# utiasSTARS/pyslam

Hardware: AMD Instinct MI355X
Metric: ms/LM-iter (Jac build + J^T J + Schur solve), stereo BA @ 500k residuals (lower is better)
Workload: dtype f64

## Files before the change

include/pyslam_hip.h:

```cpp
#ifndef PYSLAM_HIP_H
#define PYSLAM_HIP_H

#include <stdint.h>

#ifdef __cplusplus
extern "C" {
#endif

typedef struct ps_problem ps_problem;

typedef struct ps_problem_desc {
    int32_t dof;
    int32_t num_poses;
    const double*  poses;
    const int32_t* pose_rid;
    int32_t num_points;
    const double*  points;
    const int32_t* point_vid;

    int64_t num_obs;
    const int32_t* obs_pose;
    const int32_t* obs_point;
    const double*  obs_uvd;
    const int32_t* obs_grp;
// ... 138 lines not shown
                          double* dx, double* covariance );

int ps_sparse_normal_solve(int32_t m, int32_t n, const int32_t* j_row_ptr, const int32_t* j_col, const double* j_val,
                           const int32_t* jt_row_ptr, const int32_t* jt_col, const double* jt_val,
                           const double* r, const double* rhs, double tol, int32_t max_iters,
                           double* dx, int32_t* iters_out, double* relres_out);

int ps_sparse_normal_direct(int32_t m, int32_t n, const int32_t* j_row_ptr, const int32_t* j_col, const double* j_val,
                            const int32_t* jt_row_ptr, const int32_t* jt_col, const double* jt_val,
                            const double* r, const double* rhs, int32_t refine_steps, double* dx, double* relres_out);

int ps_debug_band_inverse(const double* a, int32_t ncb, int32_t dof, int32_t bw, int32_t chunk_nodes, float* ainv_out,
                          double* elapsed_us);
int ps_debug_factor_stress(const double* a, int32_t ncb, int32_t dof, int32_t bw, int32_t mode, int32_t launches, int32_t lowprio,
                           int32_t aggressor, int32_t* n_diff, int32_t* n_pivot);

int ps_ransac_transforms(const double* pts_1, const double* pts_2, int32_t batch, int32_t n, double* T_out);
int ps_ransac_cost(const double* T, int32_t num_hyp, const double* pts_1, const double* obs_2, int32_t num_pts,
                   const double* cam5, double thresh, uint8_t* masks, int32_t* counts);
int ps_ransac_frame_to_frame(const double* pts_1, const double* pts_2, const double* obs_2, int32_t num_pts,
                             const int32_t* sample_idx, int32_t num_hyp, int32_t set_size, const double* cam5,
                             double thresh, double* T_all, int32_t* counts, int32_t* best_index,
                             int32_t* best_count, double* T_best, uint8_t* best_mask);

typedef struct ps_photo ps_photo;
typedef struct ps_photo_desc {
    int32_t num_pixels;
    const double* pt_ref;
    const double* im_ref;
    const double* im_jac;
// ... 40 lines not shown
```

pyslam_amd/_native.py:

```python
import ctypes as C
import os

import numpy as np

_HERE = os.path.dirname(os.path.abspath(__file__))
LIB_PATH = os.path.join(_HERE, 'lib', 'libpyslam_hip.so')
if os.environ.get('PYSLAM_AMD_MEASURE') == '1':
    LIB_PATH = os.path.join(_HERE, 'lib', 'libpyslam_hip_measure.so')

c_i32p = C.POINTER(C.c_int32)
c_f64p = C.POINTER(C.c_double)
c_u8p = C.POINTER(C.c_uint8)
PS_NUM_STAGES = 12
STAGE_NAMES = ['landmark_pass', 'pose_pass', 'schur_pairs', 'pose_factors', 'pcg',
               'backsub', 'update', 'cost', 'iteration_total', 'cg_kernel', 'allreduce', 'pack_unpack']


class ProblemDesc(C.Structure):
    _fields_ = [
        ('dof', C.c_int32), ('num_poses', C.c_int32), ('poses', c_f64p), ('pose_rid', c_i32p),
        ('num_points', C.c_int32), ('points', c_f64p), ('point_vid', c_i32p),
        ('num_obs', C.c_int64), ('obs_pose', c_i32p), ('obs_point', c_i32p), ('obs_uvd', c_f64p),
        ('obs_grp', c_i32p),
        ('num_cams', C.c_int32), ('cams', c_f64p), ('num_stiff3', C.c_int32), ('stiff3', c_f64p),
# ... 104 lines not shown
    'ps_dense_make_tables': (C.c_int, [H, C.c_int32, C.c_int32, c_i32p, c_f64p, C.c_double, C.c_double, C.c_double]),
    'ps_dense_track': (C.c_int, [H, C.c_int32, C.c_int32, C.c_int32, c_i32p, c_i32p, C.POINTER(SolveOptions), C.c_int32,
                                 C.c_double, c_f64p, c_f64p, c_i32p, c_f64p, C.c_int32]),
    'ps_dense_level_shape': (C.c_int, [H, C.c_int32, c_i32p, c_i32p]),
    'ps_dense_read_level': (C.c_int, [H, C.c_int32, C.c_int32, C.c_int32, c_f64p]),
    'ps_dense_num_pixels': (C.c_int, [H, C.c_int32, C.c_int32, c_i32p]),
    'ps_dense_read_tables': (C.c_int, [H, C.c_int32, C.c_int32, C.c_int32, c_f64p, c_f64p, c_f64p, c_f64p]),
    'ps_dense_device_bytes': (C.c_int, [H, C.POINTER(C.c_int64)]),
    'ps_dense_normal_solve': (C.c_int, [c_f64p, c_f64p, C.c_int32, C.c_int32, c_f64p, c_f64p]),
    'ps_sparse_normal_solve': (C.c_int, [C.c_int32, C.c_int32, c_i32p, c_i32p, c_f64p, c_i32p, c_i32p, c_f64p, c_f64p, c_f64p,
                                         C.c_double, C.c_int32, c_f64p, c_i32p, c_f64p]),
    'ps_sparse_normal_direct': (C.c_int, [C.c_int32, C.c_int32, c_i32p, c_i32p, c_f64p, c_i32p, c_i32p, c_f64p, c_f64p, c_f64p,
                                          C.c_int32, c_f64p, c_f64p]),
    'ps_debug_band_inverse': (C.c_int, [c_f64p, C.c_int32, C.c_int32, C.c_int32, C.c_int32, C.POINTER(C.c_float), c_f64p]),
    'ps_debug_factor_stress': (C.c_int, [c_f64p, C.c_int32, C.c_int32, C.c_int32, C.c_int32, C.c_int32, C.c_int32, C.c_int32, c_i32p, c_i32p]),
}

_lib = None


class NativeError(RuntimeError):
    pass


def _share_torch_hip_runtime():
    import sys
    if 'torch' in sys.modules:
        return
    try:
        import importlib.util
# ... 83 lines not shown
```

pyslam_amd/csrc/ps_abi_problem.h:

```cpp


const char* ps_last_error(void) { return g_err.c_str(); }

int ps_device_count(void) {
    int n = 0;
    if (hipGetDeviceCount(&n) != hipSuccess) return 0;
    return n;
}

int ps_warm_up(void) {
    static std::once_flag once;
    static int rc = 0;
    std::call_once(once, [] {
        void* p = nullptr;
        if (hipMalloc(&p, 256) != hipSuccess) { rc = fail("hipMalloc failed (no usable HIP device?)"); return; }
        hipLaunchKernelGGL(k_zero4, dim3(1), dim3(256), 0, 0, (size_t)8, (double*)p, (size_t)0, (double*)nullptr, (size_t)0,
                           (double*)nullptr, (size_t)0, (double*)nullptr);
        double hostw[4] = {0, 0, 0, 0};
        (void)hipMemsetAsync(p, 0, 256, 0);
        (void)hipMemcpyAsync((char*)p + 128, p, 64, hipMemcpyDeviceToDevice, 0);
        (void)hipMemcpyAsync(hostw, p, sizeof(hostw), hipMemcpyDeviceToHost, 0);
        if (hipDeviceSynchronize() != hipSuccess) rc = fail("the warm-up launch failed");
        hipFree(p);
        hipFuncAttributes a;
#define PS_TOUCH(...) (void)hipFuncGetAttributes(&a, reinterpret_cast<const void*>(&__VA_ARGS__))
        PS_TOUCH(k_landmark_pass<false>); PS_TOUCH(k_landmark_pass_packed<false, false>); PS_TOUCH(k_landmark_pass_packed<false, true>); PS_TOUCH(k_backsub_packed); PS_TOUCH(k_pose_pass<false>); PS_TOUCH(k_pose_finalize); PS_TOUCH(k_schur_pairs_db<0>);
        PS_TOUCH(k_schur_combine); PS_TOUCH(k_backsub); PS_TOUCH(k_cost_reproj<false>); PS_TOUCH(k_cost_packed<false>); PS_TOUCH(k_reduce3); PS_TOUCH(k_reduce_partials);
        PS_TOUCH(k_copy2); PS_TOUCH(k_zero4); PS_TOUCH(k_lag_status_check);
        PS_TOUCH(k_block_jacobi_factor<6>); PS_TOUCH(k_scale_blocks<6>); PS_TOUCH(k_scale_blocks_p<6>); PS_TOUCH(k_rows_setup<6>);
        PS_TOUCH(k_coarse_rowsums<6>); PS_TOUCH(k_coarse_matrix<6>); PS_TOUCH(k_coarse_chol<6, true>); PS_TOUCH(k_coarse_border<6>);
        PS_TOUCH(k_coarse_mreduce<6>); PS_TOUCH(k_coarse_xbuild<6>); PS_TOUCH(k_coarse_recover<6>); PS_TOUCH(k_cg_fused_lds<6, 8>);
        PS_TOUCH(k_cg_fused<6, 8>); PS_TOUCH(k_cg_unscale<6>); PS_TOUCH(k_update_poses<6>); PS_TOUCH(k_update_points);
        PS_TOUCH(k_xcoarse_rowsums<6>); PS_TOUCH(k_xcoarse_matrix<6>); PS_TOUCH(k_band_chol<6>); PS_TOUCH(k_band_inverse); PS_TOUCH(k_band_inverse_rl<false>);
        PS_TOUCH(k_band_inverse_rl<true>); PS_TOUCH(k_bp_v); PS_TOUCH(k_bp_t); PS_TOUCH(k_bp_w); PS_TOUCH(k_bp_dense_sep); PS_TOUCH(k_bp_dense);
        PS_TOUCH(k_xcg_restrict<6>); PS_TOUCH(k_xcg_f2_coarse<6, 3>); PS_TOUCH(k_xcg_fused1<6, 8, false>); PS_TOUCH(k_xcg_fused1<6, 0, true>);
        PS_TOUCH(k_xcg_fused1<6, 2, false>); PS_TOUCH(k_xcg_fused1<6, 6, false>);
        PS_TOUCH(k_factor_pass<6>); PS_TOUCH(k_factor_assemble<6>); PS_TOUCH(k_cost_factors<6>);
        PS_TOUCH(k_factor_pass<3>); PS_TOUCH(k_factor_assemble<3>); PS_TOUCH(k_cost_factors<3>); PS_TOUCH(k_block_jacobi_factor<3>);
        PS_TOUCH(k_update_poses<3>); PS_TOUCH(k_direct_solve<6>); PS_TOUCH(k_direct_solve<3>);
        PS_TOUCH(k_motion_only_solve<false>); PS_TOUCH(k_motion_only_iteration<false>);
        PS_TOUCH(k_pcg_spmv<6>); PS_TOUCH(k_pcg_spmv<3>); PS_TOUCH(k_ldi_init); PS_TOUCH(k_ldi_update); PS_TOUCH(k_ldi_gemm); PS_TOUCH(k_ldi_mirror);
        PS_TOUCH(k_ldi_ritz); PS_TOUCH(k_ldi_seed_prep); PS_TOUCH(k_ldi_fro_total); PS_TOUCH(k_ldi_pad_identity);
        PS_TOUCH(k_ldi_scaled_dense<6>); PS_TOUCH(k_ldi_sym_unscale<6>); PS_TOUCH(k_ldi_scaled_dense<3>); PS_TOUCH(k_ldi_sym_unscale<3>);
        PS_TOUCH(k_shard_pack<6>); PS_TOUCH(k_shard_unpack<6>); PS_TOUCH(k_publish); PS_TOUCH(k_cov_rhs);
        PS_TOUCH(k_scale_blocks<3>); PS_TOUCH(k_rows_setup<3>); PS_TOUCH(k_coarse_rowsums<3>); PS_TOUCH(k_coarse_matrix<3>);
        PS_TOUCH(k_coarse_chol<3, true>); PS_TOUCH(k_coarse_border<3>); PS_TOUCH(k_coarse_mreduce<3>); PS_TOUCH(k_coarse_xbuild<3>);
        PS_TOUCH(k_coarse_recover<3>); PS_TOUCH(k_cg_fused_lds<3, 8>); PS_TOUCH(k_cg_unscale<3>);
#undef PS_TOUCH
    });
    return rc;
}

int ps_problem_destroy(ps_problem* h) {
    if (!h) return 0;
    if (h->cp_dbg) {
        long long c[8]; hipMemcpy(c, h->cp_dbg, 64, hipMemcpyDeviceToHost);
        int khz = 100000; hipDeviceGetAttribute(&khz, hipDeviceAttributeWallClockRate, 0);
        fprintf(stderr, "k_cg_persist, workgroup 0, %ld launches, us per launch: recurrences %.2f | sync %.2f | products + publish %.2f | gather %.2f "
                "(%.1f failed passes) | sync %.2f | dots + sync %.2f\n", h->cp_launches, c[0] * 1e3 / khz / h->cp_launches, c[1] * 1e3 / khz / h->cp_launches,
                c[2] * 1e3 / khz / h->cp_launches, c[3] * 1e3 / khz / h->cp_launches, (double)c[7] / h->cp_launches, c[4] * 1e3 / khz / h->cp_launches,
                c[5] * 1e3 / khz / h->cp_launches);
// ... 1058 lines not shown
```

pyslam_amd/csrc/ps_abi_small.h:

```cpp

int ps_ransac_transforms(const double* pts_1, const double* pts_2, int32_t batch, int32_t n, double* T_out) {
    if (!pts_1 || !pts_2 || !T_out || batch < 0 || n <= 0) return fail("bad argument");
    if (batch == 0) return 0;
    if (need_device()) return -1;
    const size_t nb = (size_t)batch * n * 3 * sizeof(double);
    DevBuf a, b, t;
    if (a.get(nb) || b.get(nb) || t.get((size_t)batch * 16 * sizeof(double))) return -1;
    HIP_OK(hipMemcpy(a.p, pts_1, nb, hipMemcpyHostToDevice));
    HIP_OK(hipMemcpy(b.p, pts_2, nb, hipMemcpyHostToDevice));
    hipLaunchKernelGGL(k_ransac_transforms, dim3(cdiv(batch, 64)), dim3(64), 0, 0, batch, n, a.as<double>(), b.as<double>(),
                       t.as<double>());
    HIP_OK(hipMemcpy(T_out, t.p, (size_t)batch * 16 * sizeof(double), hipMemcpyDeviceToHost));
    return 0;
}

int ps_ransac_cost(const double* T, int32_t num_hyp, const double* pts_1, const double* obs_2, int32_t num_pts,
                   const double* cam5, double thresh, uint8_t* masks, int32_t* counts) {
    if (!T || !pts_1 || !obs_2 || !cam5 || num_hyp < 0 || num_pts < 0) return fail("bad argument");
    if (num_hyp == 0) return 0;
    if (need_device()) return -1;
    DevBuf dT, dp, dobs, dcam, dcnt, dmask;
    const size_t pb = (size_t)num_pts * 3 * sizeof(double);
    if (dT.get((size_t)num_hyp * 16 * sizeof(double)) || dp.get(pb) || dobs.get(pb) || dcam.get(5 * sizeof(double)) ||
        dcnt.get((size_t)num_hyp * sizeof(int32_t)) || dmask.get((size_t)num_hyp * num_pts)) return -1;
// ... 438 lines not shown
                                    : bp->run<3>(st, bA.as<double>(), nc, bInv.as<float>(), nc, bst.as<int32_t>());
            HIP_OK(hipEventRecord(e1, st));
            if (rc) { bp.reset(); return -1; }
            if (rep == 1) { HIP_OK(hipStreamSynchronize(st)); bp.reset(); }
        }
        HIP_OK(hipStreamSynchronize(st));
    }
    HIP_OK(hipEventElapsedTime(&ms, e0, e1));
    if (elapsed_us) *elapsed_us = 1e3 * ms;
    int32_t stw[ST_NWORDS];
    HIP_OK(hipMemcpy(stw, bst.p, sizeof(stw), hipMemcpyDeviceToHost));
    HIP_OK(hipMemcpy(ainv_out, bInv.p, (size_t)nc * nc * 4, hipMemcpyDeviceToHost));
    if (stw[ST_DIAG_FAIL]) return fail("band factorisation: the matrix is not positive definite");
    return 0;
}
```

pyslam_amd/csrc/ps_abi_solver.h:

```cpp

int ps_get_info(ps_problem* h, ps_problem_info* info) {
    if (!h || !info) return fail("null argument");
    info->dof = h->D; info->num_poses = h->P; info->num_reduced = h->nr; info->num_points = h->L;
    info->num_var_points = h->nv; info->num_obs = h->N; info->num_edges = h->F; info->num_priors = 0;
    info->reduced_nnzb = h->nnzb; info->num_pairs = h->npairs;
    info->reduce_count = ((long)h->nnzb + h->nr) / 2 * h->D * h->D + (long)h->nr * h->D + 3;
    info->device_bytes = (int64_t)h->dev_bytes;
    info->cg_restarts = h->cg_fallbacks;
    info->cg_kernel_launches = h->cg_kernel_launches;
    info->ldi_solves = h->ldi_solves; info->ldi_fallbacks = h->ldi_fallbacks; info->ldi_seeds = h->ldi_seeds;
    info->xcg_fused_solves = h->xf_solves; info->xcg_fused_fallbacks = h->xf_fallbacks;
    info->cg_persist_solves = h->cp_launches; info->cg_persist_failures = h->cp_failures;
    info->cg_persist_refused = h->cp_refused; info->persist_cus = h->persist_cus;
    info->persist_cus_needed = h->cp_ok ? h->cp_cus_needed : (h->xp_ok ? h->xp_cus_needed : 0);
    info->landmark_passes_taken_over = h->prelm_used;
    info->xcg_persist4_solves = h->xp4_launches;
    return 0;
}

int ps_eval_cost(ps_problem* h, int include_all_constant, double* cost) {
    if (!h || !cost) return fail("null argument");
    if (include_all_constant && h->fuse_cost == 1 && lm_cost_possible(h)) { if (lm_cost_pass(h, h->lin_lambda, SC_COST)) return -1; }
    else if (cost_pass(h, include_all_constant, SC_COST)) return -1;
    if (read_scalars(h)) return -1;
// ... 747 lines not shown
    else if (n == "cg_ablate" || n == "schur_ablate" || n == "lm_ablate") {
        if (value != 0.0) return fail(n + ": timing experiments exist in the measurement build only (__graft_entry__.build_measure(), PYSLAM_AMD_MEASURE=1)");
    }
#endif
    else if (n == "schur_pipeline") h->schur_pipeline = value != 0.0;
    else if (n == "schur_mode") {
        if (value != 0.0 && value != 1.0) return fail("schur_mode must be 0 (gather kernels) or 1 (pose-stationary kernel)");
        if (value == 0.0 && !h->gather_lists) return fail("schur_mode 0: the gather kernels' pair lists were not built for this handle (create it under PS_SCHUR_MODE=0 or 2)");
        h->schur_mode = (int)value;
    }
    else if (n == "schur_stream") { if (value != 0.0 && !h->st_tiles) return fail("schur_stream: the streaming lists were not built for this problem"); h->use_stream = value != 0.0; }
    else if (n == "coarse_lag") h->coarse_lag = value != 0.0;
    else if (n == "cg_force_restart") h->cg_force_restart = value != 0.0;
    else if (n == "xcg_restrict_fused") h->xcg_rt = value != 0;
    else if (n == "band_chol") { h->band_chol = value != 0; h->lci_next = -1; }
    else if (n == "lm_packed") h->lm_packed = value != 0;
    else if (n == "pose_async") h->pose_async = (int)value;
    else if (n == "pose_xcd") h->pose_xcd = value != 0;
    else if (n == "xcg_persist4") h->xcg_persist4 = value != 0;
    else if (n == "cg_pipelined") { if (value != 0 && value != 1 && value != 2) return fail("cg_pipelined must be 0, 1 or 2"); h->cg_pipelined = (int)value; }
    else if (n == "fuse_cost") h->fuse_cost = (int)value;
    else if (n == "sync_refactor") h->sync_refactor = value != 0;
    else if (n == "hold_across_steps") h->hold_across_steps = value != 0;
    else if (n == "band_part") { h->band_part = value != 0; h->lci_next = -1; }
    else if (n == "band_part_chunk") { if (value < 0 || value > 4096) return fail("band_part_chunk must be 0 (automatic) .. 4096 nodes"); h->band_part_m = (int)value; h->lci_next = -1; }
    else if (n == "coarse_auto_hold") h->xcg_auto_hold = value != 0;
    else if (n == "coarse_adaptive_hold") h->xcg_adaptive_hold = value != 0;
    else if (n == "xcg_fused") { if (value != 0 && value != 1 && value != 2) return fail("xcg_fused must be 0, 1 or 2"); h->xcg_fused = (int)value; }
    else if (n == "lagged_inverse") { h->ldi_enable = value != 0; if (!h->ldi_enable) { h->ldi_cur = -1; if (h->ldi_state != 1) h->ldi_state = 0; } relook_path(h); }
    else if (n == "ldi_max_unknowns") { if (value < 0 || value > PS_LDI_MAXN) return fail("ldi_max_unknowns out of range (0 .. 3328)"); h->ldi_max_n = (int)value; relook_path(h); }
// ... 114 lines not shown
```

pyslam_amd/csrc/ps_core.hip:

```cpp
#include <hip/hip_runtime.h>

#include <algorithm>
#include <array>
#include <map>
#include <atomic>
#include <chrono>
#include <thread>
#include <climits>
#include <cmath>
#include <cstdio>
#include <cstring>
#include <memory>
#include <mutex>
#include <string>
#include <vector>

#include "pyslam_hip.h"
#include "ps_kernels.h"
#include "ps_ransac.h"
#include "ps_photo.h"
#include "ps_k_dense.h"
#include "ps_sparse.h"

namespace {
// ... 208 lines not shown
    bool side_pending = false;
    int coarse_lag = 1;
    hipStream_t side = nullptr;
    int side_cus = 0;
    hipEvent_t ev_ac = nullptr, ev_chol = nullptr, ev_acdone = nullptr;
    unsigned long long* chk_sums = nullptr; int chk_nsum = 0;
    double *chk_Ac = nullptr, *chk_BSZ = nullptr, *chk_Ac_side = nullptr; int32_t* chk_cnt = nullptr; size_t chk_bsz_n = 0;
    bool acdone_pending = false;
    int32_t* lag_status = nullptr;
    double* Mc = nullptr;
    bool mc_active = false;
    bool coarse_built = false;
    bool coarse_clamped = false;
    int cg_ablate = 0, schur_ablate = 0, lm_ablate = 0;
    int schur_pipeline = 1;
    int max_pose_obs = 0;
    int mo_fused = 1;
    double* mo_partials = nullptr;
    bool status_clean = true;
    int direct_fused = ps_env("PS_DIRECT_3LAUNCH") ? 0 : 1;
    int direct_max = 90;
    double *dA = nullptr, *dLi = nullptr, *dLiT = nullptr;
    int big_chol = 1;
    int explicit_ok = 1;
    bool cg_explicit = false;
    int xcg_refresh_every = 1;
    long xcg_lag_count = 0;
    int xcg_auto_hold = 1, xcg_held = 0;
    int xcg_adaptive_hold = 1;
    int xcg_its_ref = 0, xcg_good_held = 0;
// ... 300 lines not shown
```

pyslam_amd/csrc/ps_host_cg.h:

```cpp

namespace {

struct StageTimer {
    ps_problem* h;
    int stage;
    hipEvent_t a = nullptr, b = nullptr;
    int slot = -1;
    StageTimer(ps_problem* h_, int st, int level = 2) : h(h_), stage(st) {
        if (h->profiling < level) return;
        if (h->profiling == 1 && h->prof_every > 1 &&
            h->prof_tick % h->prof_every != (st == PS_ST_CG_KERNEL ? h->prof_every / 2 : 0)) return;
        if (h->ev_used + 2 > h->ev_pool.size()) {
            for (int i = 0; i < 64; ++i) { hipEvent_t e; hipEventCreate(&e); h->ev_pool.push_back(e); }
        }
        slot = (int)h->ev_used;
        a = h->ev_pool[h->ev_used++];
        b = h->ev_pool[h->ev_used++];
        hipEventRecord(a, h->stream);
    }
    void stop() {
        if (!a) return;
        hipEventRecord(b, h->stream);
        h->pending.push_back({stage, slot});
        a = nullptr;
// ... 480 lines not shown
    if (h->side_pending) { HIP_OK(hipStreamWaitEvent(h->stream, h->ev_chol, 0)); h->side_pending = false; }
    h->acdone_pending = false;
    h->lci_next = -1; h->lci_cur = 0; h->xcg_tag[0] = h->xcg_tag[1] = -1.0;
    if (ensure_cg_buffers(h, h->nr_aug, h->nnzb_aug)) return -1;
    HIP_OK(hipMemsetAsync(h->Saug, 0, (size_t)h->nnzb_aug * D * D * sizeof(double), h->stream));
    return 0;
}

inline void copy_doubles(hipStream_t st, double* dst, const double* src, size_t n) {
    if (!n) return;
    hipLaunchKernelGGL(k_copy2, dim3((unsigned)std::min<size_t>(2048, cdiv((long)n, 256))), dim3(256), 0, st, n, src, dst, (size_t)0,
                       (const double*)nullptr, (double*)nullptr);
}

template <int D>
int coarse_factor(ps_problem* h, hipStream_t st, int buf, int32_t* stat) {
    const int nc = h->nc, ncb = h->ncb;
    if (nc <= 90) {
        const size_t chol_lds = 2 * (size_t)nc * nc * sizeof(double);
        if (ensure_dynamic_lds((const void*)k_coarse_chol<D, true>, (size_t)(chol_lds))) return -1;
        hipLaunchKernelGGL((k_coarse_chol<D, true>), dim3(1), dim3(1024), chol_lds, st, ncb, h->Ac, h->Lci2[buf],
                           h->LciT2[buf], stat, nullptr);
    } else if (h->big_chol) {
        double* A = h->chol_scratch;
        double* Tinv = A + (size_t)nc * nc;
        copy_doubles(st, A, h->Ac, (size_t)nc * nc);
        const int nsteps = cdiv(nc, PS_BC_W);
        for (int s2 = 0; s2 < nsteps; ++s2) {
            const int j0 = s2 * PS_BC_W, w = std::min(PS_BC_W, nc - j0), m = nc - j0 - w;
            hipLaunchKernelGGL(k_bchol_panel, dim3(std::max(1, cdiv((long)m * w, 1024))), dim3(256), 0, st, nc, j0, A,
                               Tinv + (size_t)s2 * PS_BC_W * PS_BC_W, stat);
            if (m > 0) {
                const int nt = cdiv(m, 32);
                hipLaunchKernelGGL(k_bchol_update, dim3(nt * (nt + 1) / 2), dim3(256), 0, st, nc, j0, w, A);
            }
        }
        const bool dense_out = nc > PS_BI_S0 && !h->cg_explicit;
// ... 646 lines not shown
```

pyslam_amd/csrc/ps_host_iteration.h:

```cpp

namespace {

inline bool xcg_ac_on_main() { static const bool v = ps_env("PS_XCG_AC_MAIN") != nullptr; return v; }

template <int D>
void xcg_assemble_ac(ps_problem* h, hipStream_t st) {
    const int nr = h->nr, ncb = h->ncb;
    hipLaunchKernelGGL(k_xcoarse_rowsums<D>, dim3(nr), dim3(256), (size_t)(h->max_row_ents + 1) * D * D * sizeof(double), st,
                       nr, h->ent_ptr, h->ent_q, h->ent_lo, h->ent_hi, h->acol_idx, h->pnode, h->pw0, h->pw1, h->SB, h->Bmat, h->BSZ);
    hipLaunchKernelGGL(k_xcoarse_matrix<D>, dim3(cdiv((long)ncb * ncb * D * D, 256)), dim3(256), 0, st,
                       ncb, h->seg_ptr, h->seg_ent, h->seg_row, h->pnode, h->pw0, h->pw1, h->BSZ, h->Ac);
}

template <int D>
void xcg_launch(ps_problem* h, double tol, int count);

template <int D>
int xcg_setup(ps_problem* h, int max_iters, bool allow_lag) {
    const int nr = h->nr, ncb = h->ncb, nc = h->nc;
    if (max_iters + 2 > h->hist_cap) return fail("pcg max_iters exceeds the history buffer (4096)");
    if (h->acdone_pending) { HIP_OK(hipStreamWaitEvent(h->stream, h->ev_acdone, 0)); h->acdone_pending = false; }
    hipLaunchKernelGGL(k_block_jacobi_factor<D>, dim3(cdiv(nr, 4)), dim3(256), 0, h->stream, nr, h->diag_slot,
                       h->S, h->Linv, h->status, h->g, h->cg_r[0], h->cg_w[0], h->cg_s[0], h->cg_p, h->cg_xh,
                       h->poses, h->pose_of_rid, h->coarse_basis, h->Bmat, h->bgv);
// ... 336 lines not shown
int direct_solve_enqueue(ps_problem* h) {
    const int nr = h->nr, n = nr * D;
    if (h->direct_fused) {
        const size_t lds = ((size_t)n * n + 2 * (size_t)n + (size_t)nr * D * D) * sizeof(double);
        if (ensure_dynamic_lds((const void*)k_direct_solve<D>, lds)) return -1;
        static const int nt_env = ps_env("PS_DIRECT_THREADS") ? atoi(ps_env("PS_DIRECT_THREADS")) : 0;
        const int nthreads = nt_env > 0 ? nt_env : 1024;
        hipLaunchKernelGGL(k_direct_solve<D>, dim3(1), dim3(nthreads), lds, h->stream, nr, h->nnzb, h->brow_of, h->col_idx, h->S, h->g, h->x,
                           h->status, h->scalars);
        h->cg_launched = 0;
        return 0;
    }
    if (!h->dA && (h->alloc(&h->dA, (size_t)n * n) || h->alloc(&h->dLi, (size_t)n * n) || h->alloc(&h->dLiT, (size_t)n * n)))
        return -1;
    hipLaunchKernelGGL(k_bsr_to_dense<D>, dim3(1), dim3(256), 0, h->stream, nr, h->nnzb, h->brow_of, h->col_idx, h->S, h->dA);
    const size_t chol_lds = 2 * (size_t)n * n * sizeof(double);
    if (ensure_dynamic_lds((const void*)k_coarse_chol<D, true>, (size_t)(chol_lds))) return -1;
    hipLaunchKernelGGL((k_coarse_chol<D, true>), dim3(1), dim3(1024), chol_lds, h->stream, nr, h->dA, h->dLi, h->dLiT,
                       h->status, nullptr);
    hipLaunchKernelGGL(k_direct_apply<D>, dim3(1), dim3(256), 0, h->stream, n, h->dLi, h->dLiT, h->g, h->x, h->status,
                       h->scalars);
    h->cg_launched = 0;
    return 0;
}

int solve_reduced(ps_problem* h, double tol, int max_iters, int* iters, double* relres) {
    if (h->nr == 0) { if (iters) *iters = 0; if (relres) *relres = 0.0; return 0; }
    StageTimer t(h, PS_ST_PCG);
    if (use_direct(h)) {
        if (h->D == 6 ? direct_solve_enqueue<6>(h) : direct_solve_enqueue<3>(h)) return -1;
        if (read_scalars(h)) return -1;
        return cg_report(h, iters, relres);
    }
    if (h->pcg_variant == 1) {
// ... 161 lines not shown
```

pyslam_amd/csrc/ps_k_coarse.h:

```cpp
#pragma once


PS_DEV double coarse_weight(int j, int q, const int32_t* __restrict__ pnode,
                            const double* __restrict__ pw0, const double* __restrict__ pw1) {
    return (pnode[j] == q) ? pw0[j] : pw1[j];
}

template <int D>
__global__ __launch_bounds__(256) void k_coarse_rowsums(
    int nr, int ncb, const int32_t* __restrict__ run_lo, const int32_t* __restrict__ run_hi,
    const int32_t* __restrict__ acol_idx, const int32_t* __restrict__ pnode,
    const double* __restrict__ pw0, const double* __restrict__ pw1,
    const double* __restrict__ SB ,
    double* __restrict__ SZ, const double* __restrict__ Bmat, double* __restrict__ BSZ )
{
    constexpr int DD = D * D;
    extern __shared__ double srow[];
    const int i = blockIdx.x, nslot = ncb * DD;
    double* sBi = srow + nslot;
    if (threadIdx.x < DD) sBi[threadIdx.x] = Bmat[(size_t)i * DD + threadIdx.x];
    for (int t = threadIdx.x; t < nslot; t += blockDim.x) {
        const int q = t / DD, e = t % DD;
        const int k0 = run_lo[i * ncb + q], k1 = run_hi[i * ncb + q];
        double acc = 0.0;
// ... 68 lines not shown
    const int32_t* __restrict__ seg_row, const int32_t* __restrict__ pnode, const double* __restrict__ pw0,
    const double* __restrict__ pw1, const double* __restrict__ BSZ, double* __restrict__ Ac)
{
    constexpr int DD = D * D;
    const int nc = ncb * D;
    const int t = blockIdx.x * blockDim.x + threadIdx.x;
    if (t >= ncb * ncb * DD) return;
    const int e = t % DD, q2 = (t / DD) % ncb, q = t / (DD * ncb);
    double acc = 0.0;
    for (int s = seg_ptr[q * ncb + q2]; s < seg_ptr[q * ncb + q2 + 1]; ++s)
        acc += coarse_weight(seg_row[s], q, pnode, pw0, pw1) * BSZ[(size_t)seg_ent[s] * DD + e];
    Ac[(size_t)(q * D + e / D) * nc + q2 * D + e % D] = acc;
}

template <int D, bool IN_LDS>
__global__ __launch_bounds__(1024) void k_coarse_chol(int ncb, const double* __restrict__ A,
                                                       double* __restrict__ Li, double* __restrict__ LiT,
                                                       int32_t* __restrict__ status, double* gscratch)
{
    constexpr int DD = D * D;
    extern __shared__ __attribute__((aligned(16))) double sm[];
    const int nc = ncb * D;
    double* sL = IN_LDS ? sm : gscratch;
    double* sX = sL + nc * nc;
    __shared__ double sRl[64 * 6];
    const int t = threadIdx.x, nt = blockDim.x;
    for (int k = t; k < nc * nc; k += nt) { sL[k] = A[k]; sX[k] = 0.0; }
    auto factor_diag = [&](int J) {
        double a[D][D], rl[D];
        bool ok = true;
#pragma unroll
        for (int r = 0; r < D; ++r)
#pragma unroll
            for (int c = 0; c <= r; ++c) a[r][c] = sL[(J * D + r) * nc + J * D + c];
#pragma unroll
        for (int jj = 0; jj < D; ++jj) {
            double d = a[jj][jj];
#pragma unroll
            for (int k = 0; k < jj; ++k) d -= a[jj][k] * a[jj][k];
            if (!(d > 0.0)) { ok = false; d = 1.0; }
            rl[jj] = ps_rsqrt(d);
            a[jj][jj] = d * rl[jj];
#pragma unroll
            for (int r = jj + 1; r < D; ++r) {
                double v = a[r][jj];
#pragma unroll
                for (int k = 0; k < jj; ++k) v -= a[r][k] * a[jj][k];
                a[r][jj] = v * rl[jj];
            }
        }
        if (!ok) atomicAdd(&status[ST_DIAG_FAIL], 1);
#pragma unroll
        for (int r = 0; r < D; ++r) {
            sRl[J * D + r] = rl[r];
#pragma unroll
            for (int c = 0; c < D; ++c) sL[(J * D + r) * nc + J * D + c] = c <= r ? a[r][c] : 0.0;
        }
    };
    __syncthreads();
    if (t == 0) factor_diag(0);
    for (int J = 0; J < ncb; ++J) {
        __syncthreads();
        const int m = ncb - J - 1;
        for (int row = t; row < m * D; row += nt) {
            double* ar = sL + ((J + 1) * D + row) * nc + J * D;
            double x[D];
#pragma unroll
            for (int c = 0; c < D; ++c) {
                double v = ar[c];
#pragma unroll
                for (int k = 0; k < c; ++k) v -= x[k] * sL[(J * D + c) * nc + J * D + k];
                x[c] = v * sRl[J * D + c];
            }
#pragma unroll
            for (int c = 0; c < D; ++c) ar[c] = x[c];
        }
        __syncthreads();
        if (m == 0) break;
        if (t < 64) {
            if (t < DD) {
                const int a = t / D, b2 = t % D;
                double v = 0.0;
#pragma unroll
                for (int k = 0; k < D; ++k) v += sL[((J + 1) * D + a) * nc + J * D + k] * sL[((J + 1) * D + b2) * nc + J * D + k];
                sL[((J + 1) * D + a) * nc + (J + 1) * D + b2] -= v;
            }
            __builtin_amdgcn_wave_barrier();
            if (t == 0) factor_diag(J + 1);
        } else {
            for (int idx = t - 64; idx < m * m * DD; idx += nt - 64) {
                const int blk = idx / DD, e = idx % DD, a = e / D, b2 = e % D;
                const int I = J + 1 + blk / m, K = J + 1 + blk % m;
                if (K > I || (I == J + 1 && K == J + 1)) continue;
                double v = 0.0;
#pragma unroll
                for (int k = 0; k < D; ++k) v += sL[(I * D + a) * nc + J * D + k] * sL[(K * D + b2) * nc + J * D + k];
                sL[(I * D + a) * nc + K * D + b2] -= v;
            }
        }
    }
    __syncthreads();
    for (int k = t; k < ncb * D; k += nt) {
        const int R = k / D, c = k % D;
        double col[D];
#pragma unroll
        for (int r = 0; r < D; ++r) {
            double v = (r == c) ? 1.0 : 0.0;
#pragma unroll
            for (int q = 0; q < r; ++q) v -= (q >= c) ? sL[(R * D + r) * nc + R * D + q] * col[q] : 0.0;
            col[r] = (r >= c) ? v * sRl[R * D + r] : 0.0;
            sX[(R * D + r) * nc + R * D + c] = col[r];
        }
    }
    constexpr int NEX = IN_LDS ? 9 : 1;
    short ei[NEX], ej[NEX];
// ... 23 lines not shown
    };
    for (int sg = 1, lg = 1; sg < ncb; sg *= 2, ++lg) {
        __syncthreads();
        if (IN_LDS) {
#pragma unroll
            for (int u = 0; u < NEX; ++u) if (ei[u] >= 0) t_entry(ei[u], ej[u], sg, lg);
        } else for (int idx = t; idx < nc * nc; idx += nt) t_entry(idx / nc, idx % nc, sg, lg);
        __syncthreads();
        if (IN_LDS) {
#pragma unroll
            for (int u = 0; u < NEX; ++u) if (ei[u] >= 0) x_entry(ei[u], ej[u], sg, lg);
        } else for (int idx = t; idx < nc * nc; idx += nt) x_entry(idx / nc, idx % nc, sg, lg);
    }
    __syncthreads();
    for (int k = t; k < nc * nc; k += nt) {
        const int r = k / nc, c = k % nc;
        const double v = (c <= r) ? sX[k] : 0.0;
        Li[k] = v;
        LiT[(size_t)c * nc + r] = v;
    }
}

#define PS_BC_W 24
__global__ __launch_bounds__(256) void k_bchol_panel(
    int nc, int j0, double* __restrict__ A ,
    double* __restrict__ Tinv ,
    int32_t* __restrict__ status)
{
    __shared__ double sD[PS_BC_W * PS_BC_W], sI[PS_BC_W * PS_BC_W];
    const int t = threadIdx.x, w = min(PS_BC_W, nc - j0);
// ... 595 lines not shown
```

pyslam_amd/device.py:

```python
import ctypes as C

import numpy as np

from pyslam_amd import _native as nat


class DeviceProblem:
    def __init__(self, lp, stream=None, extra_pairs=None):
        lib = nat.require_gpu()
        self._lib = lib
        self.lp = lp
        self.dof = lp.dof
        d = nat.ProblemDesc()
        keep = []
        params_res = nat.is_resident(lp.poses)
        tables_res = nat.is_resident(lp.pose_rid)
        if params_res != nat.is_resident(lp.points):
            raise TypeError('poses and points must both be host arrays or both device tensors')
        d.flags = (nat.PS_DESC_DEVICE_PARAMS if params_res else 0) | (nat.PS_DESC_DEVICE_TABLES if tables_res else 0)

        def conv(a, np_dtype, want_res, to_ptr):
            if nat.is_resident(a) != want_res:
                raise TypeError('mixed host / device tables (ps_problem_desc.flags is per class: parameters, everything else)')
            if not want_res:
# ... 283 lines not shown
    cov = np.zeros((n, n)) if want_covariance else None
    nat.check(lib.ps_dense_normal_solve(nat.f64p(J), nat.f64p(r), m, n, nat.f64p(dx), nat.f64p(cov)))
    return (dx, cov) if want_covariance else dx


def band_inverse(A, ncb, dof, bw, chunk_nodes=0):
    lib = nat.require_gpu()
    A = np.ascontiguousarray(A, dtype=np.float64)
    n = ncb * dof
    assert A.shape == (n, n)
    out = np.zeros((n, n), dtype=np.float32)
    us = C.c_double(0.0)
    nat.check(lib.ps_debug_band_inverse(nat.f64p(A), ncb, dof, bw, chunk_nodes, out.ctypes.data_as(C.POINTER(C.c_float)),
                                        C.cast(C.byref(us), nat.c_f64p)))
    return out, us.value


class NotConverged(nat.NativeError):
    """The CG of the host-evaluated path stopped at max_iters with a residual too large to use."""


def sparse_normal_solve(J, r=None, rhs=None, tol=1e-12, max_iters=10000, accept=1e-6):
    lib = nat.require_gpu()
    J = J.tocsr()
    J.sort_indices()
    Jt = J.T.tocsr()
    Jt.sort_indices()
    m, n = J.shape
    a = [np.ascontiguousarray(x, dtype=t) for x, t in ((J.indptr, np.int32), (J.indices, np.int32), (J.data, np.float64),
                                                        (Jt.indptr, np.int32), (Jt.indices, np.int32), (Jt.data, np.float64))]
# ... 250 lines not shown
```

Baseline: 0.3034.

## Add fused coarse Cholesky kernel with precomputed thread mapping and fast inverse

```diff
diff --git a/include/pyslam_hip.h b/include/pyslam_hip.h
--- a/include/pyslam_hip.h
+++ b/include/pyslam_hip.h
@@ -176,6 +176,8 @@
                           double* elapsed_us);
 int ps_debug_factor_stress(const double* a, int32_t ncb, int32_t dof, int32_t bw, int32_t mode, int32_t launches, int32_t lowprio,
                            int32_t aggressor, int32_t* n_diff, int32_t* n_pivot);
+int ps_debug_coarse_chol(const double* a, int32_t ncb, int32_t dof, int32_t fused, int32_t repeats, double* li_out,
+                         int32_t* diag_fail, double* elapsed_us);
 
 int ps_ransac_transforms(const double* pts_1, const double* pts_2, int32_t batch, int32_t n, double* T_out);
 int ps_ransac_cost(const double* T, int32_t num_hyp, const double* pts_1, const double* obs_2, int32_t num_pts,
diff --git a/pyslam_amd/_native.py b/pyslam_amd/_native.py
--- a/pyslam_amd/_native.py
+++ b/pyslam_amd/_native.py
@@ -142,6 +142,7 @@
                                           C.c_int32, c_f64p, c_f64p]),
     'ps_debug_band_inverse': (C.c_int, [c_f64p, C.c_int32, C.c_int32, C.c_int32, C.c_int32, C.POINTER(C.c_float), c_f64p]),
     'ps_debug_factor_stress': (C.c_int, [c_f64p, C.c_int32, C.c_int32, C.c_int32, C.c_int32, C.c_int32, C.c_int32, C.c_int32, c_i32p, c_i32p]),
+    'ps_debug_coarse_chol': (C.c_int, [c_f64p, C.c_int32, C.c_int32, C.c_int32, C.c_int32, c_f64p, c_i32p, c_f64p]),
 }
 
 _lib = None
diff --git a/pyslam_amd/csrc/ps_abi_problem.h b/pyslam_amd/csrc/ps_abi_problem.h
--- a/pyslam_amd/csrc/ps_abi_problem.h
+++ b/pyslam_amd/csrc/ps_abi_problem.h
@@ -28,7 +28,7 @@
         PS_TOUCH(k_schur_combine); PS_TOUCH(k_backsub); PS_TOUCH(k_cost_reproj<false>); PS_TOUCH(k_cost_packed<false>); PS_TOUCH(k_reduce3); PS_TOUCH(k_reduce_partials);
         PS_TOUCH(k_copy2); PS_TOUCH(k_zero4); PS_TOUCH(k_lag_status_check);
         PS_TOUCH(k_block_jacobi_factor<6>); PS_TOUCH(k_scale_blocks<6>); PS_TOUCH(k_scale_blocks_p<6>); PS_TOUCH(k_rows_setup<6>);
-        PS_TOUCH(k_coarse_rowsums<6>); PS_TOUCH(k_coarse_matrix<6>); PS_TOUCH(k_coarse_chol<6, true>); PS_TOUCH(k_coarse_border<6>);
+        PS_TOUCH(k_coarse_rowsums<6>); PS_TOUCH(k_coarse_matrix<6>); PS_TOUCH(k_coarse_chol<6, true>); PS_TOUCH(k_coarse_chol_fs<6, false>); PS_TOUCH(k_coarse_border<6>);
         PS_TOUCH(k_coarse_mreduce<6>); PS_TOUCH(k_coarse_xbuild<6>); PS_TOUCH(k_coarse_recover<6>); PS_TOUCH(k_cg_fused_lds<6, 8>);
         PS_TOUCH(k_cg_fused<6, 8>); PS_TOUCH(k_cg_unscale<6>); PS_TOUCH(k_update_poses<6>); PS_TOUCH(k_update_points);
         PS_TOUCH(k_xcoarse_rowsums<6>); PS_TOUCH(k_xcoarse_matrix<6>); PS_TOUCH(k_band_chol<6>); PS_TOUCH(k_band_inverse); PS_TOUCH(k_band_inverse_rl<false>);
@@ -44,7 +44,7 @@
         PS_TOUCH(k_ldi_scaled_dense<6>); PS_TOUCH(k_ldi_sym_unscale<6>); PS_TOUCH(k_ldi_scaled_dense<3>); PS_TOUCH(k_ldi_sym_unscale<3>);
         PS_TOUCH(k_shard_pack<6>); PS_TOUCH(k_shard_unpack<6>); PS_TOUCH(k_publish); PS_TOUCH(k_cov_rhs);
         PS_TOUCH(k_scale_blocks<3>); PS_TOUCH(k_rows_setup<3>); PS_TOUCH(k_coarse_rowsums<3>); PS_TOUCH(k_coarse_matrix<3>);
-        PS_TOUCH(k_coarse_chol<3, true>); PS_TOUCH(k_coarse_border<3>); PS_TOUCH(k_coarse_mreduce<3>); PS_TOUCH(k_coarse_xbuild<3>);
+        PS_TOUCH(k_coarse_chol<3, true>); PS_TOUCH(k_coarse_chol_fs<3, false>); PS_TOUCH(k_coarse_border<3>); PS_TOUCH(k_coarse_mreduce<3>); PS_TOUCH(k_coarse_xbuild<3>);
         PS_TOUCH(k_coarse_recover<3>); PS_TOUCH(k_cg_fused_lds<3, 8>); PS_TOUCH(k_cg_unscale<3>);
 #undef PS_TOUCH
     });
diff --git a/pyslam_amd/csrc/ps_abi_small.h b/pyslam_amd/csrc/ps_abi_small.h
--- a/pyslam_amd/csrc/ps_abi_small.h
+++ b/pyslam_amd/csrc/ps_abi_small.h
@@ -476,3 +476,36 @@
     if (stw[ST_DIAG_FAIL]) return fail("band factorisation: the matrix is not positive definite");
     return 0;
 }
+
+int ps_debug_coarse_chol(const double* a, int32_t ncb, int32_t dof, int32_t fused, int32_t repeats, double* li_out,
+                         int32_t* diag_fail, double* elapsed_us) {
+    if (!a || !li_out || !diag_fail || ncb <= 0 || (dof != 3 && dof != 6) || ncb * dof > 90 || repeats < 1) return fail("bad argument");
+    if (need_device()) return -1;
+    const int nc = ncb * dof;
+    DevBuf bA, bLi, bLiT, bst;
+    if (bA.get((size_t)nc * nc * 8) || bLi.get((size_t)nc * nc * 8) || bLiT.get((size_t)nc * nc * 8) || bst.get(ST_NWORDS * 4)) return -1;
+    HIP_OK(hipMemcpy(bA.p, a, (size_t)nc * nc * 8, hipMemcpyHostToDevice));
+    hipStream_t st = 0;
+    hipEvent_t e0, e1;
+    HIP_OK(hipEventCreate(&e0)); HIP_OK(hipEventCreate(&e1));
+    struct Ev { hipEvent_t a, b; ~Ev() { hipEventDestroy(a); hipEventDestroy(b); } } evs{e0, e1};
+    auto launch = [&]() -> int {
+        return dof == 6 ? launch_coarse_chol_lds<6>(fused, st, ncb, bA.as<double>(), bLi.as<double>(), bLiT.as<double>(), bst.as<int32_t>())
+                        : launch_coarse_chol_lds<3>(fused, st, ncb, bA.as<double>(), bLi.as<double>(), bLiT.as<double>(), bst.as<int32_t>());
+    };
+    HIP_OK(hipMemsetAsync(bst.p, 0, ST_NWORDS * 4, st));
+    if (launch()) return -1;
+    HIP_OK(hipStreamSynchronize(st));
+    int32_t stw[ST_NWORDS];
+    HIP_OK(hipMemcpy(stw, bst.p, sizeof(stw), hipMemcpyDeviceToHost));
+    HIP_OK(hipMemcpy(li_out, bLi.p, (size_t)nc * nc * 8, hipMemcpyDeviceToHost));
+    *diag_fail = stw[ST_DIAG_FAIL];
+    HIP_OK(hipEventRecord(e0, st));
+    for (int k = 0; k < repeats; ++k) if (launch()) return -1;
+    HIP_OK(hipEventRecord(e1, st));
+    HIP_OK(hipStreamSynchronize(st));
+    float ms = 0.f;
+    HIP_OK(hipEventElapsedTime(&ms, e0, e1));
+    if (elapsed_us) *elapsed_us = 1e3 * ms / repeats;
+    return 0;
+}
diff --git a/pyslam_amd/csrc/ps_abi_solver.h b/pyslam_amd/csrc/ps_abi_solver.h
--- a/pyslam_amd/csrc/ps_abi_solver.h
+++ b/pyslam_amd/csrc/ps_abi_solver.h
@@ -785,6 +785,7 @@
     else if (n == "cg_force_restart") h->cg_force_restart = value != 0.0;
     else if (n == "xcg_restrict_fused") h->xcg_rt = value != 0;
     else if (n == "band_chol") { h->band_chol = value != 0; h->lci_next = -1; }
+    else if (n == "setup_fused") h->setup_fused = (int)value;
     else if (n == "lm_packed") h->lm_packed = value != 0;
     else if (n == "pose_async") h->pose_async = (int)value;
     else if (n == "pose_xcd") h->pose_xcd = value != 0;
diff --git a/pyslam_amd/csrc/ps_core.hip b/pyslam_amd/csrc/ps_core.hip
--- a/pyslam_amd/csrc/ps_core.hip
+++ b/pyslam_amd/csrc/ps_core.hip
@@ -246,6 +246,7 @@
     bool coarse_clamped = false;
     int cg_ablate = 0, schur_ablate = 0, lm_ablate = 0;
     int schur_pipeline = 1;
+    int setup_fused = 1;
     int max_pose_obs = 0;
     int mo_fused = 1;
     double* mo_partials = nullptr;
diff --git a/pyslam_amd/csrc/ps_host_cg.h b/pyslam_amd/csrc/ps_host_cg.h
--- a/pyslam_amd/csrc/ps_host_cg.h
+++ b/pyslam_amd/csrc/ps_host_cg.h
@@ -518,13 +518,26 @@
 }
 
 template <int D>
+int launch_coarse_chol_lds(int fused, hipStream_t st, int ncb, const double* A, double* Li, double* LiT, int32_t* status) {
+    const size_t lds = 2 * (size_t)(ncb * D) * (ncb * D) * sizeof(double);
+    if (fused == 2) {
+        if (ensure_dynamic_lds((const void*)k_coarse_chol_fs<D, true>, lds)) return -1;
+        hipLaunchKernelGGL((k_coarse_chol_fs<D, true>), dim3(1), dim3(1024), lds, st, ncb, A, Li, LiT, status);
+    } else if (fused) {
+        if (ensure_dynamic_lds((const void*)k_coarse_chol_fs<D, false>, lds)) return -1;
+        hipLaunchKernelGGL((k_coarse_chol_fs<D, false>), dim3(1), dim3(1024), lds, st, ncb, A, Li, LiT, status);
+    } else {
+        if (ensure_dynamic_lds((const void*)k_coarse_chol<D, true>, lds)) return -1;
+        hipLaunchKernelGGL((k_coarse_chol<D, true>), dim3(1), dim3(1024), lds, st, ncb, A, Li, LiT, status, nullptr);
+    }
+    return 0;
+}
+
+template <int D>
 int coarse_factor(ps_problem* h, hipStream_t st, int buf, int32_t* stat) {
     const int nc = h->nc, ncb = h->ncb;
     if (nc <= 90) {
-        const size_t chol_lds = 2 * (size_t)nc * nc * sizeof(double);
-        if (ensure_dynamic_lds((const void*)k_coarse_chol<D, true>, (size_t)(chol_lds))) return -1;
-        hipLaunchKernelGGL((k_coarse_chol<D, true>), dim3(1), dim3(1024), chol_lds, st, ncb, h->Ac, h->Lci2[buf],
-                           h->LciT2[buf], stat, nullptr);
+        if (launch_coarse_chol_lds<D>(h->setup_fused, st, ncb, h->Ac, h->Lci2[buf], h->LciT2[buf], stat)) return -1;
     } else if (h->big_chol) {
         double* A = h->chol_scratch;
         double* Tinv = A + (size_t)nc * nc;
diff --git a/pyslam_amd/csrc/ps_host_iteration.h b/pyslam_amd/csrc/ps_host_iteration.h
--- a/pyslam_amd/csrc/ps_host_iteration.h
+++ b/pyslam_amd/csrc/ps_host_iteration.h
@@ -374,10 +374,7 @@
     if (!h->dA && (h->alloc(&h->dA, (size_t)n * n) || h->alloc(&h->dLi, (size_t)n * n) || h->alloc(&h->dLiT, (size_t)n * n)))
         return -1;
     hipLaunchKernelGGL(k_bsr_to_dense<D>, dim3(1), dim3(256), 0, h->stream, nr, h->nnzb, h->brow_of, h->col_idx, h->S, h->dA);
-    const size_t chol_lds = 2 * (size_t)n * n * sizeof(double);
-    if (ensure_dynamic_lds((const void*)k_coarse_chol<D, true>, (size_t)(chol_lds))) return -1;
-    hipLaunchKernelGGL((k_coarse_chol<D, true>), dim3(1), dim3(1024), chol_lds, h->stream, nr, h->dA, h->dLi, h->dLiT,
-                       h->status, nullptr);
+    if (launch_coarse_chol_lds<D>(h->setup_fused, h->stream, nr, h->dA, h->dLi, h->dLiT, h->status)) return -1;
     hipLaunchKernelGGL(k_direct_apply<D>, dim3(1), dim3(256), 0, h->stream, n, h->dLi, h->dLiT, h->g, h->x, h->status,
                        h->scalars);
     h->cg_launched = 0;
diff --git a/pyslam_amd/csrc/ps_k_coarse.h b/pyslam_amd/csrc/ps_k_coarse.h
--- a/pyslam_amd/csrc/ps_k_coarse.h
+++ b/pyslam_amd/csrc/ps_k_coarse.h
@@ -106,91 +106,11 @@
 }
 
 template <int D, bool IN_LDS>
-__global__ __launch_bounds__(1024) void k_coarse_chol(int ncb, const double* __restrict__ A,
-                                                       double* __restrict__ Li, double* __restrict__ LiT,
-                                                       int32_t* __restrict__ status, double* gscratch)
-{
-    constexpr int DD = D * D;
-    extern __shared__ __attribute__((aligned(16))) double sm[];
+PS_DEV void coarse_chol_inverse_out(int ncb, const double* sL, double* sX, const double* sRl, double* __restrict__ Li,
+                                    double* __restrict__ LiT)
+{
     const int nc = ncb * D;
-    double* sL = IN_LDS ? sm : gscratch;
-    double* sX = sL + nc * nc;
-    __shared__ double sRl[64 * 6];
     const int t = threadIdx.x, nt = blockDim.x;
-    for (int k = t; k < nc * nc; k += nt) { sL[k] = A[k]; sX[k] = 0.0; }
-    auto factor_diag = [&](int J) {
-        double a[D][D], rl[D];
-        bool ok = true;
-#pragma unroll
-        for (int r = 0; r < D; ++r)
-#pragma unroll
-            for (int c = 0; c <= r; ++c) a[r][c] = sL[(J * D + r) * nc + J * D + c];
-#pragma unroll
-        for (int jj = 0; jj < D; ++jj) {
-            double d = a[jj][jj];
-#pragma unroll
-            for (int k = 0; k < jj; ++k) d -= a[jj][k] * a[jj][k];
-            if (!(d > 0.0)) { ok = false; d = 1.0; }
-            rl[jj] = ps_rsqrt(d);
-            a[jj][jj] = d * rl[jj];
-#pragma unroll
-            for (int r = jj + 1; r < D; ++r) {
-                double v = a[r][jj];
-#pragma unroll
-                for (int k = 0; k < jj; ++k) v -= a[r][k] * a[jj][k];
-                a[r][jj] = v * rl[jj];
-            }
-        }
-        if (!ok) atomicAdd(&status[ST_DIAG_FAIL], 1);
-#pragma unroll
-        for (int r = 0; r < D; ++r) {
-            sRl[J * D + r] = rl[r];
-#pragma unroll
-            for (int c = 0; c < D; ++c) sL[(J * D + r) * nc + J * D + c] = c <= r ? a[r][c] : 0.0;
-        }
-    };
-    __syncthreads();
-    if (t == 0) factor_diag(0);
-    for (int J = 0; J < ncb; ++J) {
-        __syncthreads();
-        const int m = ncb - J - 1;
-        for (int row = t; row < m * D; row += nt) {
-            double* ar = sL + ((J + 1) * D + row) * nc + J * D;
-            double x[D];
-#pragma unroll
-            for (int c = 0; c < D; ++c) {
-                double v = ar[c];
-#pragma unroll
-                for (int k = 0; k < c; ++k) v -= x[k] * sL[(J * D + c) * nc + J * D + k];
-                x[c] = v * sRl[J * D + c];
-            }
-#pragma unroll
-            for (int c = 0; c < D; ++c) ar[c] = x[c];
-        }
-        __syncthreads();
-        if (m == 0) break;
-        if (t < 64) {
-            if (t < DD) {
-                const int a = t / D, b2 = t % D;
-                double v = 0.0;
-#pragma unroll
-                for (int k = 0; k < D; ++k) v += sL[((J + 1) * D + a) * nc + J * D + k] * sL[((J + 1) * D + b2) * nc + J * D + k];
-                sL[((J + 1) * D + a) * nc + (J + 1) * D + b2] -= v;
-            }
-            __builtin_amdgcn_wave_barrier();
-            if (t == 0) factor_diag(J + 1);
-        } else {
-            for (int idx = t - 64; idx < m * m * DD; idx += nt - 64) {
-                const int blk = idx / DD, e = idx % DD, a = e / D, b2 = e % D;
-                const int I = J + 1 + blk / m, K = J + 1 + blk % m;
-                if (K > I || (I == J + 1 && K == J + 1)) continue;
-                double v = 0.0;
-#pragma unroll
-                for (int k = 0; k < D; ++k) v += sL[(I * D + a) * nc + J * D + k] * sL[(K * D + b2) * nc + J * D + k];
-                sL[(I * D + a) * nc + K * D + b2] -= v;
-            }
-        }
-    }
     __syncthreads();
     for (int k = t; k < ncb * D; k += nt) {
         const int R = k / D, c = k % D;
@@ -244,6 +164,290 @@
     }
     __syncthreads();
     for (int k = t; k < nc * nc; k += nt) {
+        const int r = k / nc, c = k % nc;
+        const double v = (c <= r) ? sX[k] : 0.0;
+        Li[k] = v;
+        LiT[(size_t)c * nc + r] = v;
+    }
+}
+
+template <int D>
+PS_DEV void coarse_chol_inverse_out_fast(int ncb, const double* sL, double* sX, const double* sRl, double* __restrict__ Li,
+                                         double* __restrict__ LiT)
+{
+    const int nc = ncb * D;
+    const int t = threadIdx.x, nt = blockDim.x;
+    __syncthreads();
+    for (int k = t; k < ncb * D; k += nt) {
+        const int R = k / D, c = k % D;
+        double col[D];
+#pragma unroll
+        for (int r = 0; r < D; ++r) {
+            double v = (r == c) ? 1.0 : 0.0;
+#pragma unroll
+            for (int q = 0; q < r; ++q) v -= (q >= c) ? sL[(R * D + r) * nc + R * D + q] * col[q] : 0.0;
+            col[r] = (r >= c) ? v * sRl[R * D + r] : 0.0;
+            sX[(R * D + r) * nc + R * D + c] = col[r];
+        }
+    }
+    for (int sg = 1; sg < ncb; sg *= 2) {
+        const int w = sg * D, npair = (ncb + 2 * sg - 1) / (2 * sg), nslot = npair * w * w;
+        __syncthreads();
+        for (int u = t; u < nslot; u += nt) {
+            const int p = u / (w * w), r = (u / w) % w, c = u % w;
+            const int i = (2 * p + 1) * w + r, jj = 2 * p * w + c, k1 = (2 * p + 1) * w;
+            if (i >= nc) continue;
+            const double* li = sL + i * nc;
+            double v = 0.0;
+            int k = jj;
+            for (; k + 4 <= k1; k += 4) {
+                const double a0 = li[k], a1 = li[k + 1], a2 = li[k + 2], a3 = li[k + 3];
+                const double b0 = sX[k * nc + jj], b1 = sX[(k + 1) * nc + jj], b2 = sX[(k + 2) * nc + jj], b3 = sX[(k + 3) * nc + jj];
+                v += a0 * b0; v += a1 * b1; v += a2 * b2; v += a3 * b3;
+            }
+            for (; k < k1; ++k) v += li[k] * sX[k * nc + jj];
+            sX[jj * nc + i] = v;
+        }
+        __syncthreads();
+        for (int u = t; u < nslot; u += nt) {
+            const int p = u / (w * w), r = (u / w) % w, c = u % w;
+            const int i = (2 * p + 1) * w + r, jj = 2 * p * w + c, k0 = (2 * p + 1) * w;
+            if (i >= nc) continue;
+            const double* xi = sX + i * nc;
+            const double* tj = sX + jj * nc;
+            double v = 0.0;
+            int k = k0;
+            for (; k + 4 <= i + 1; k += 4) {
+                const double a0 = xi[k], a1 = xi[k + 1], a2 = xi[k + 2], a3 = xi[k + 3];
+                const double b0 = tj[k], b1 = tj[k + 1], b2 = tj[k + 2], b3 = tj[k + 3];
+                v -= a0 * b0; v -= a1 * b1; v -= a2 * b2; v -= a3 * b3;
+            }
+            for (; k <= i; ++k) v -= xi[k] * tj[k];
+            sX[i * nc + jj] = v;
+        }
+    }
+    __syncthreads();
+    for (int k = t; k < nc * nc; k += nt) {
+        const int r = k / nc, c = k % nc;
+        const double v = (c <= r) ? sX[k] : 0.0;
+        Li[k] = v;
+        LiT[(size_t)c * nc + r] = v;
+    }
+}
+
+template <int D, bool IN_LDS>
+__global__ __launch_bounds__(1024) void k_coarse_chol(int ncb, const double* __restrict__ A,
+                                                       double* __restrict__ Li, double* __restrict__ LiT,
+                                                       int32_t* __restrict__ status, double* gscratch)
+{
+    constexpr int DD = D * D;
+    extern __shared__ __attribute__((aligned(16))) double sm[];
+    const int nc = ncb * D;
+    double* sL = IN_LDS ? sm : gscratch;
+    double* sX = sL + nc * nc;
+    __shared__ double sRl[64 * 6];
+    const int t = threadIdx.x, nt = blockDim.x;
+    for (int k = t; k < nc * nc; k += nt) { sL[k] = A[k]; sX[k] = 0.0; }
+    auto factor_diag = [&](int J) {
+        double a[D][D], rl[D];
+        bool ok = true;
+#pragma unroll
+        for (int r = 0; r < D; ++r)
+#pragma unroll
+            for (int c = 0; c <= r; ++c) a[r][c] = sL[(J * D + r) * nc + J * D + c];
+#pragma unroll
+        for (int jj = 0; jj < D; ++jj) {
+            double d = a[jj][jj];
+#pragma unroll
+            for (int k = 0; k < jj; ++k) d -= a[jj][k] * a[jj][k];
+            if (!(d > 0.0)) { ok = false; d = 1.0; }
+            rl[jj] = ps_rsqrt(d);
+            a[jj][jj] = d * rl[jj];
+#pragma unroll
+            for (int r = jj + 1; r < D; ++r) {
+                double v = a[r][jj];
+#pragma unroll
+                for (int k = 0; k < jj; ++k) v -= a[r][k] * a[jj][k];
+                a[r][jj] = v * rl[jj];
+            }
+        }
+        if (!ok) atomicAdd(&status[ST_DIAG_FAIL], 1);
+#pragma unroll
+        for (int r = 0; r < D; ++r) {
+            sRl[J * D + r] = rl[r];
+#pragma unroll
+            for (int c = 0; c < D; ++c) sL[(J * D + r) * nc + J * D + c] = c <= r ? a[r][c] : 0.0;
+        }
+    };
+    __syncthreads();
+    if (t == 0) factor_diag(0);
+    for (int J = 0; J < ncb; ++J) {
+        __syncthreads();
+        const int m = ncb - J - 1;
+        for (int row = t; row < m * D; row += nt) {
+            double* ar = sL + ((J + 1) * D + row) * nc + J * D;
+            double x[D];
+#pragma unroll
+            for (int c = 0; c < D; ++c) {
+                double v = ar[c];
+#pragma unroll
+                for (int k = 0; k < c; ++k) v -= x[k] * sL[(J * D + c) * nc + J * D + k];
+                x[c] = v * sRl[J * D + c];
+            }
+#pragma unroll
+            for (int c = 0; c < D; ++c) ar[c] = x[c];
+        }
+        __syncthreads();
+        if (m == 0) break;
+        if (t < 64) {
+            if (t < DD) {
+                const int a = t / D, b2 = t % D;
+                double v = 0.0;
+#pragma unroll
+                for (int k = 0; k < D; ++k) v += sL[((J + 1) * D + a) * nc + J * D + k] * sL[((J + 1) * D + b2) * nc + J * D + k];
+                sL[((J + 1) * D + a) * nc + (J + 1) * D + b2] -= v;
+            }
+            __builtin_amdgcn_wave_barrier();
+            if (t == 0) factor_diag(J + 1);
+        } else {
+            for (int idx = t - 64; idx < m * m * DD; idx += nt - 64) {
+                const int blk = idx / DD, e = idx % DD, a = e / D, b2 = e % D;
+                const int I = J + 1 + blk / m, K = J + 1 + blk % m;
+                if (K > I || (I == J + 1 && K == J + 1)) continue;
+                double v = 0.0;
+#pragma unroll
+                for (int k = 0; k < D; ++k) v += sL[(I * D + a) * nc + J * D + k] * sL[(K * D + b2) * nc + J * D + k];
+                sL[(I * D + a) * nc + K * D + b2] -= v;
+            }
+        }
+    }
+    coarse_chol_inverse_out<D, IN_LDS>(ncb, sL, sX, sRl, Li, LiT);
+}
+
+template <int D, bool INV_FS>
+__global__ __launch_bounds__(1024) void k_coarse_chol_fs(int ncb, const double* __restrict__ A, double* __restrict__ Li,
+                                                         double* __restrict__ LiT, int32_t* __restrict__ status)
+{
+    constexpr int NCB_MAX = 90 / D, NT = 1024, NW = NT - 64;
+    constexpr int NU = ((NCB_MAX - 1) * NCB_MAX * D + NW - 1) / NW;
+    extern __shared__ __attribute__((aligned(16))) double sm[];
+    const int nc = ncb * D;
+    double* sL = sm;
+    double* sX = sL + nc * nc;
+    __shared__ double sRl[96];
+    const int t = threadIdx.x;
+    for (int k = t; k < nc * nc; k += NT) {
+        sL[k] = A[k];
+        sX[k] = (INV_FS && k / nc == k % nc) ? 1.0 : 0.0;
+    }
+    auto factor_diag = [&](int J) {
+        double a[D][D], rl[D];
+        bool ok = true;
+#pragma unroll
+        for (int r = 0; r < D; ++r)
+#pragma unroll
+            for (int c = 0; c <= r; ++c) a[r][c] = sL[(J * D + r) * nc + J * D + c];
+#pragma unroll
+        for (int jj = 0; jj < D; ++jj) {
+            double d = a[jj][jj];
+#pragma unroll
+            for (int k = 0; k < jj; ++k) d -= a[jj][k] * a[jj][k];
+            if (!(d > 0.0)) { ok = false; d = 1.0; }
+            rl[jj] = ps_rsqrt(d);
+            a[jj][jj] = d * rl[jj];
+#pragma unroll
+            for (int r = jj + 1; r < D; ++r) {
+                double v = a[r][jj];
+#pragma unroll
+                for (int k = 0; k < jj; ++k) v -= a[r][k] * a[jj][k];
+                a[r][jj] = v * rl[jj];
+            }
+        }
+        if (!ok) atomicAdd(&status[ST_DIAG_FAIL], 1);
+#pragma unroll
+        for (int r = 0; r < D; ++r) {
+            sRl[J * D + r] = rl[r];
+#pragma unroll
+            for (int c = 0; c < D; ++c) sL[(J * D + r) * nc + J * D + c] = c <= r ? a[r][c] : 0.0;
+        }
+    };
+    short uI[NU], uK[NU], ua[NU];
+#pragma unroll
+    for (int s = 0; s < NU; ++s) {
+        const int u = t - 64 + s * NW;
+        const bool ok = t >= 64 && u < (ncb - 1) * ncb * D;
+        uI[s] = ok ? (short)(u / (ncb * D)) : (short)NCB_MAX;
+        uK[s] = (short)((u / D) % ncb);
+        ua[s] = (short)(u % D);
+    }
+    __syncthreads();
+    if (t == 0) factor_diag(0);
+    for (int J = 0; J < ncb; ++J) {
+        __syncthreads();
+        const int m = ncb - J - 1;
+        const double* Ljj = sL + (J * D) * nc + J * D;
+        if (t < m * D) {
+            double* ar = sL + ((J + 1) * D + t) * nc + J * D;
+            double x[D];
+#pragma unroll
+            for (int c = 0; c < D; ++c) {
+                double v = ar[c];
+#pragma unroll
+                for (int k = 0; k < c; ++k) v -= x[k] * Ljj[c * nc + k];
+                x[c] = v * sRl[J * D + c];
+            }
+#pragma unroll
+            for (int c = 0; c < D; ++c) ar[c] = x[c];
+        } else if (INV_FS && t >= 128 && t < 128 + (J + 1) * D) {
+            double* xc = sX + (J * D) * nc + (t - 128);
+            double x[D];
+#pragma unroll
+            for (int r = 0; r < D; ++r) {
+                double v = xc[r * nc];
+#pragma unroll
+                for (int q = 0; q < r; ++q) v -= Ljj[r * nc + q] * x[q];
+                x[r] = v * sRl[J * D + r];
+            }
+#pragma unroll
+            for (int r = 0; r < D; ++r) xc[r * nc] = x[r];
+        }
+        __syncthreads();
+        if (m == 0) break;
+        if (t < 64) {
+            if (t < D * D) {
+                const int a = t / D, b2 = t % D;
+                double v = 0.0;
+#pragma unroll
+                for (int k = 0; k < D; ++k) v += sL[((J + 1) * D + a) * nc + J * D + k] * sL[((J + 1) * D + b2) * nc + J * D + k];
+                sL[((J + 1) * D + a) * nc + (J + 1) * D + b2] -= v;
+            }
+            __builtin_amdgcn_wave_barrier();
+            if (t == 0) factor_diag(J + 1);
+        } else {
+#pragma unroll
+            for (int s = 0; s < NU; ++s) {
+                const int I = J + 1 + uI[s], K = uK[s];
+                if (I >= ncb || K > I || (I == J + 1 && K == J + 1) || (!INV_FS && K <= J)) continue;
+                const double* lr = sL + (I * D + ua[s]) * nc + J * D;
+                double l[D];
+#pragma unroll
+                for (int k = 0; k < D; ++k) l[k] = lr[k];
+                const bool upd_a = K > J;
+                const double* y = upd_a ? sL + (K * D) * nc + J * D : sX + (J * D) * nc + K * D;
+                const int sk = upd_a ? 1 : nc, sb = upd_a ? nc : 1;
+                double* dst = (upd_a ? sL : sX) + (I * D + ua[s]) * nc + K * D;
+#pragma unroll
+                for (int b2 = 0; b2 < D; ++b2) {
+                    double v = 0.0;
+#pragma unroll
+                    for (int k = 0; k < D; ++k) v += l[k] * y[b2 * sb + k * sk];
+                    dst[b2] -= v;
+                }
+            }
+        }
+    }
+    if (!INV_FS) { coarse_chol_inverse_out_fast<D>(ncb, sL, sX, sRl, Li, LiT); return; }
+    for (int k = t; k < nc * nc; k += NT) {
         const int r = k / nc, c = k % nc;
         const double v = (c <= r) ? sX[k] : 0.0;
         Li[k] = v;
diff --git a/pyslam_amd/device.py b/pyslam_amd/device.py
--- a/pyslam_amd/device.py
+++ b/pyslam_amd/device.py
@@ -321,6 +321,19 @@
     nat.check(lib.ps_debug_band_inverse(nat.f64p(A), ncb, dof, bw, chunk_nodes, out.ctypes.data_as(C.POINTER(C.c_float)),
                                         C.cast(C.byref(us), nat.c_f64p)))
     return out, us.value
+
+
+def coarse_chol_inverse(A, ncb, dof, fused=1, repeats=1):
+    lib = nat.require_gpu()
+    A = np.ascontiguousarray(A, dtype=np.float64)
+    n = ncb * dof
+    assert A.shape == (n, n)
+    out = np.zeros((n, n))
+    fails = C.c_int32(0)
+    us = C.c_double(0.0)
+    nat.check(lib.ps_debug_coarse_chol(nat.f64p(A), ncb, dof, int(fused), int(repeats), nat.f64p(out),
+                                       C.cast(C.byref(fails), nat.c_i32p), C.cast(C.byref(us), nat.c_f64p)))
+    return out, fails.value, us.value
 
 
 class NotConverged(nat.NativeError):
```

New measurement: 0.3010, median of 6. Within noise of the previous version (-0.8%).
